# haosulab/ActiveZero

Measured on AMD Instinct MI355X. Metric: stereo pairs/sec (540x960, D=192) fwd+bwd, higher is better.
Workload: dtype f32; 1 GPU; configs[1]: PSMNet 540x960 (padded to 544 rows) D=192 fwd+bwd+Adam, supervised disparity loss, batch 4 per GPU; global_batch=4, height=540, width=960, maxdisp=192, parallelism=dp1

## Files before the change

### activezero_amd/csrc/az_conv3d_c1.hip

```cpp
#include "az_common.h"

#define C1_TH 8
#define C1_TW 32
#define C1_VS 36
#define C1_GP 36
typedef float c1_f2 __attribute__((ext_vector_type(2)));
#define C1_FMA2(a, b, c) __builtin_elementwise_fma(a, b, c)


#define C1F_TH 8
#define C1F_TW 16
template <int CTRL>
__device__ __forceinline__ float c1_dpp_add(float v) {
    return v + __builtin_bit_cast(float, __builtin_amdgcn_update_dpp(0, __builtin_bit_cast(int, v), CTRL, 0xf, 0xf, true));
}
__global__ void __launch_bounds__(256)
c1_fwd_kernel(float *__restrict__ out, const float *__restrict__ in, const float *__restrict__ w,
              const float *__restrict__ addend, const float *__restrict__ in_scale,
              const float *__restrict__ in_shift, int D, int H, int W, int tiles_x, int dseg) {
    constexpr int SX = C1F_TW + 2, SY = C1F_TH + 2;
    __shared__ __attribute__((aligned(16))) float slab[SY * SX * C1_VS];
    const int tx0 = (blockIdx.x % tiles_x) * C1F_TW, ty0 = (blockIdx.x / tiles_x) * C1F_TH;
    const int d0 = blockIdx.y * dseg, d1 = min(d0 + dseg, D), b = blockIdx.z;
    const int cp = threadIdx.x & 15, grp = threadIdx.x >> 4;
    const int ly = grp >> 1, lx0 = (grp & 1) * 8;
    const int oh = ty0 + ly;
    c1_f2 wp[27];
#pragma unroll
    for (int t = 0; t < 27; ++t) wp[t] = c1_f2{w[(cp * 2 + 0) * 27 + t], w[(cp * 2 + 1) * 27 + t]};
    c1_f2 a_prev[8], a_cur[8], a_next[8];
#pragma unroll
    for (int j = 0; j < 8; ++j) { a_prev[j] = c1_f2{0.f, 0.f}; a_cur[j] = c1_f2{0.f, 0.f}; a_next[j] = c1_f2{0.f, 0.f}; }
    constexpr int NQ = SY * SX * 8, NLD = (NQ + 255) / 256;
    float4 pre[NLD];
    const bool affine = in_scale != nullptr;
    float4 isc = make_float4(1.f, 1.f, 1.f, 1.f), ish = make_float4(0.f, 0.f, 0.f, 0.f);
    if (affine) {
        isc = reinterpret_cast<const float4 *>(in_scale)[threadIdx.x & 7];
        ish = reinterpret_cast<const float4 *>(in_shift)[threadIdx.x & 7];
    }
    unsigned okbits = 0;
    auto issue = [&](int id) {
        okbits = 0;
#pragma unroll
        for (int it = 0; it < NLD; ++it) {
            const int q = threadIdx.x + 256 * it, v = q >> 3, part = q & 7;
            const int sy = v / SX, sx = v - sy * SX;
            const int ih = ty0 - 1 + sy, iw = tx0 - 1 + sx;
            pre[it] = make_float4(0.f, 0.f, 0.f, 0.f);
            if (q < NQ && id >= 0 && id < D && ih >= 0 && ih < H && iw >= 0 && iw < W) {
                pre[it] = *reinterpret_cast<const float4 *>(
                    in + ((((size_t)b * D + id) * H + ih) * W + iw) * 32 + part * 4);
                okbits |= 1u << it;
            }
        }
    };
    issue(d0 - 1);
    for (int id = d0 - 1; id <= d1; ++id) {
        if (id >= 0 && id < D) {
            __syncthreads();
#pragma unroll
            for (int it = 0; it < NLD; ++it) {
                const int q = threadIdx.x + 256 * it;
                float4 v = pre[it];
                if (affine && ((okbits >> it) & 1u)) {
                    v.x = fmaxf(fmaf(v.x, isc.x, ish.x), 0.f); v.y = fmaxf(fmaf(v.y, isc.y, ish.y), 0.f);
                    v.z = fmaxf(fmaf(v.z, isc.z, ish.z), 0.f); v.w = fmaxf(fmaf(v.w, isc.w, ish.w), 0.f);
                }
                if (q < NQ) *reinterpret_cast<float4 *>(&slab[(q >> 3) * C1_VS + (q & 7) * 4]) = v;
            }
            __syncthreads();
        }
        if (id < d1) issue(id + 1);
        if (id >= 0 && id < D) {
#pragma unroll
            for (int kh = 0; kh < 3; ++kh) {
                c1_f2 r[10];
                const float *row = &slab[((ly + kh) * SX + lx0) * C1_VS + cp * 2];
#pragma unroll
                for (int i = 0; i < 10; ++i) {
                    const float2 x = *reinterpret_cast<const float2 *>(row + i * C1_VS);
                    r[i] = c1_f2{x.x, x.y};
                }
#pragma unroll
                for (int kw = 0; kw < 3; ++kw)
#pragma unroll
                    for (int j = 0; j < 8; ++j) {
                        a_next[j] = C1_FMA2(r[j + kw], wp[kh * 3 + kw], a_next[j]);
                        a_cur[j] = C1_FMA2(r[j + kw], wp[9 + kh * 3 + kw], a_cur[j]);
                        a_prev[j] = C1_FMA2(r[j + kw], wp[18 + kh * 3 + kw], a_prev[j]);
                    }
            }
        }
        const int od = id - 1;
        if (od >= d0 && od < d1) {
            float mine = 0.f;
#pragma unroll
            for (int j = 0; j < 8; ++j) {
                float v = a_prev[j][0] + a_prev[j][1];
                v = c1_dpp_add<0xB1>(v);
                v = c1_dpp_add<0x4E>(v);
                v = c1_dpp_add<0x141>(v);
                v = c1_dpp_add<0x140>(v);
                mine = (cp == j) ? v : mine;
            }
            const int ow = tx0 + lx0 + cp;
            if (cp < 8 && oh < H && ow < W) {
                const size_t o = (((size_t)b * D + od) * H + oh) * W + ow;
                out[o] = addend ? mine + addend[o] : mine;
            }
        }
#pragma unroll
        for (int j = 0; j < 8; ++j) { a_prev[j] = a_cur[j]; a_cur[j] = a_next[j]; a_next[j] = c1_f2{0.f, 0.f}; }
    }
}

__device__ __forceinline__ void c1_load_gtile(float *gt, const float *__restrict__ gout, int b,
                                              int od, int ty0, int tx0, int D, int H, int W) {
    constexpr int SX = C1_TW + 2, SY = C1_TH + 2;
    for (int q = threadIdx.x; q < 3 * SY * SX; q += 256) {
        const int sx = q % SX;
        const int r = q / SX;
        const int sy = r % SY, sd = r / SY;
        const int gd = od - 1 + sd, gh = ty0 - 1 + sy, gw = tx0 - 1 + sx;
        gt[r * C1_GP + sx] = (gd >= 0 && gd < D && gh >= 0 && gh < H && gw >= 0 && gw < W)
                                 ? gout[(((size_t)b * D + gd) * H + gh) * W + gw] : 0.f;
    }
}
__device__ __forceinline__ void c1_row6(float (&r)[6], const float *gt, int pd, int sy, int lx0) {
    const float *row = static_cast<const float *>(__builtin_assume_aligned(gt + (pd * (C1_TH + 2) + sy) * C1_GP + lx0, 16));
    const float4 a = *reinterpret_cast<const float4 *>(row);
    const float2 c = *reinterpret_cast<const float2 *>(row + 4);
    r[0] = a.x; r[1] = a.y; r[2] = a.z; r[3] = a.w; r[4] = c.x; r[5] = c.y;
}

__global__ void __launch_bounds__(256)
c1_dgrad_kernel(float *__restrict__ gin, const float *__restrict__ gout,
                const float *__restrict__ w, int D, int H, int W, int tiles_x) {
    constexpr int SY = C1_TH + 2;
    __shared__ __attribute__((aligned(16))) float gt[3 * SY * C1_GP];
    const int tx0 = (blockIdx.x % tiles_x) * C1_TW, ty0 = (blockIdx.x / tiles_x) * C1_TH;
    const int od = blockIdx.y, b = blockIdx.z;
    c1_load_gtile(gt, gout, b, od, ty0, tx0, D, H, W);
    const int cp = threadIdx.x & 15, grp = threadIdx.x >> 4;
    c1_f2 wp[27];
#pragma unroll
    for (int t = 0; t < 27; ++t) wp[t] = c1_f2{w[(cp * 2 + 0) * 27 + t], w[(cp * 2 + 1) * 27 + t]};
    __syncthreads();
#pragma unroll 1
    for (int p = 0; p < C1_TH * C1_TW / 128; ++p) {
        const int gi = p * 16 + grp, ly = gi >> 2, lx0 = (gi & 3) * 8;
        const int oh = ty0 + ly;
        c1_f2 acc[8];
#pragma unroll
        for (int j = 0; j < 8; ++j) acc[j] = c1_f2{0.f, 0.f};
#pragma unroll
        for (int kd = 0; kd < 3; ++kd)
#pragma unroll
            for (int kh = 0; kh < 3; ++kh) {
                float r[12];
                {
                    const float *row = static_cast<const float *>(__builtin_assume_aligned(
                        gt + ((2 - kd) * SY + ly + 2 - kh) * C1_GP + lx0, 16));
                    const float4 a = *reinterpret_cast<const float4 *>(row);
                    const float4 c = *reinterpret_cast<const float4 *>(row + 4);
                    const float2 e = *reinterpret_cast<const float2 *>(row + 8);
                    r[0] = a.x; r[1] = a.y; r[2] = a.z; r[3] = a.w; r[4] = c.x; r[5] = c.y; r[6] = c.z; r[7] = c.w;
                    r[8] = e.x; r[9] = e.y;
                }
#pragma unroll
                for (int kw = 0; kw < 3; ++kw) {
                    const int t = (kd * 3 + kh) * 3 + kw;
#pragma unroll
                    for (int j = 0; j < 8; ++j) {
                        const c1_f2 g2 = {r[j + 2 - kw], r[j + 2 - kw]};
                        acc[j] = C1_FMA2(g2, wp[t], acc[j]);
                    }
                }
            }
#pragma unroll
        for (int j = 0; j < 8; ++j) asm volatile("" : "+v"(acc[j]));
        if (oh < H) {
            float *dst = gin + ((((size_t)b * D + od) * H + oh) * W + tx0 + lx0) * 32 + cp * 2;
#pragma unroll
            for (int j = 0; j < 8; ++j)
                if (tx0 + lx0 + j < W) *reinterpret_cast<float2 *>(dst + j * 32) = make_float2(acc[j][0], acc[j][1]);
        }
    }
}

__global__ void __launch_bounds__(256)
c1_wgrad_kernel(float *__restrict__ gw, const float *__restrict__ in,
                const float *__restrict__ gout, const float *__restrict__ in_scale,
                const float *__restrict__ in_shift, int D, int H, int W, int tiles_x, int tiles_y,
                long long ntiles) {
    constexpr int SY = C1_TH + 2;
    __shared__ __attribute__((aligned(16))) float gt[3 * SY * C1_GP];
    __shared__ float red[864];
    for (int q = threadIdx.x; q < 864; q += 256) red[q] = 0.f;
    const int quad = threadIdx.x & 7, grp = threadIdx.x >> 3;
    const bool affine = in_scale != nullptr;
    float4 isc = make_float4(1.f, 1.f, 1.f, 1.f), ish = make_float4(0.f, 0.f, 0.f, 0.f);
    if (affine) {
        isc = reinterpret_cast<const float4 *>(in_scale)[quad];
        ish = reinterpret_cast<const float4 *>(in_shift)[quad];
    }
    c1_f2 a01[27], a23[27];
#pragma unroll
    for (int t = 0; t < 27; ++t) { a01[t] = c1_f2{0.f, 0.f}; a23[t] = c1_f2{0.f, 0.f}; }
    for (long long item = blockIdx.x; item < ntiles; item += gridDim.x) {
        long long r = item;
        const int tx0 = (int)(r % tiles_x) * C1_TW; r /= tiles_x;
        const int ty0 = (int)(r % tiles_y) * C1_TH; r /= tiles_y;
        const int od = (int)(r % D);
        const int b = (int)(r / D);
        __syncthreads();
        c1_load_gtile(gt, gout, b, od, ty0, tx0, D, H, W);
        __syncthreads();
#pragma unroll 1
        for (int p = 0; p < C1_TH * C1_TW / 128; ++p) {
            const int gi = p * 32 + grp, ly = gi >> 3, lx0 = (gi & 7) * 4;
            const int ih = ty0 + ly;
            c1_f2 x01[4], x23[4];
            const float *src = in + ((((size_t)b * D + od) * H + ih) * W + tx0 + lx0) * 32 + quad * 4;
#pragma unroll
            for (int j = 0; j < 4; ++j) {
                float4 x = make_float4(0.f, 0.f, 0.f, 0.f);
                if (ih < H && tx0 + lx0 + j < W) {
                    x = *reinterpret_cast<const float4 *>(src + j * 32);
                    if (affine) {
                        x.x = fmaxf(fmaf(x.x, isc.x, ish.x), 0.f); x.y = fmaxf(fmaf(x.y, isc.y, ish.y), 0.f);
                        x.z = fmaxf(fmaf(x.z, isc.z, ish.z), 0.f); x.w = fmaxf(fmaf(x.w, isc.w, ish.w), 0.f);
                    }
                }
                x01[j] = c1_f2{x.x, x.y}; x23[j] = c1_f2{x.z, x.w};
            }
#pragma unroll
            for (int kd = 0; kd < 3; ++kd)
#pragma unroll
                for (int kh = 0; kh < 3; ++kh) {
                    float r[6];
                    c1_row6(r, gt, 2 - kd, ly + 2 - kh, lx0);
#pragma unroll
                    for (int kw = 0; kw < 3; ++kw) {
                        const int t = (kd * 3 + kh) * 3 + kw;
#pragma unroll
                        for (int j = 0; j < 4; ++j) {
                            const c1_f2 g2 = {r[j + 2 - kw], r[j + 2 - kw]};
                            a01[t] = C1_FMA2(g2, x01[j], a01[t]);
                            a23[t] = C1_FMA2(g2, x23[j], a23[t]);
                        }
                    }
                }
        }
    }
#pragma unroll
    for (int c = 0; c < 4; ++c)
#pragma unroll
        for (int t = 0; t < 27; ++t) {
            float v = (c < 2 ? a01[t] : a23[t])[c & 1];
            v += __shfl_xor(v, 8); v += __shfl_xor(v, 16); v += __shfl_xor(v, 32);
            if ((threadIdx.x & 63) < 8) atomicAdd(&red[(quad * 4 + c) * 27 + t], v);
        }
    __syncthreads();
    for (int q = threadIdx.x; q < 864; q += 256) atomicAdd(&gw[q], red[q]);
}

static int c1_check(int B, int D, int H, int W) {
    if (!(B > 0 && D > 0 && H > 0 && W > 0)) return AZ_EINVAL;
    if (B > 65535 || D > 65535) return AZ_EUNSUPPORTED;
    return AZ_OK;
}

extern "C" int az_conv3d_c1_fwd(float *logits, const float *in, const float *w,
                                const float *addend, const float *in_scale, const float *in_shift, int B, int D,
                                int H, int W, void *stream) {
    AZ_REQUIRE_PTR(logits); AZ_REQUIRE_PTR(in); AZ_REQUIRE_PTR(w);
    if ((in_scale == nullptr) != (in_shift == nullptr)) return AZ_EINVAL;
    if (int e = c1_check(B, D, H, W)) return e;
    const int tiles_x = (W + C1F_TW - 1) / C1F_TW, tiles_y = (H + C1F_TH - 1) / C1F_TH;
    int best = 1;
    long long best_cost = -1;
    for (int nseg = 1; nseg <= D; ++nseg) {
        const int dseg = (D + nseg - 1) / nseg;
        const long long blocks = (long long)tiles_x * tiles_y * B * ((D + dseg - 1) / dseg);
        const long long cost = ((blocks + 767) / 768) * (dseg + 2);
        if (best_cost < 0 || cost < best_cost) { best_cost = cost; best = dseg; }
    }
    hipLaunchKernelGGL(c1_fwd_kernel, dim3(tiles_x * tiles_y, (D + best - 1) / best, B), dim3(256), 0,
                       az_stream(stream), logits, in, w, addend, in_scale, in_shift, D, H, W, tiles_x, best);
    return az_launch_status();
}

extern "C" int az_conv3d_c1_dgrad(float *grad_in, const float *grad_logits, const float *w,
                                  int B, int D, int H, int W, void *stream) {
    AZ_REQUIRE_PTR(grad_in); AZ_REQUIRE_PTR(grad_logits); AZ_REQUIRE_PTR(w);
    if (int e = c1_check(B, D, H, W)) return e;
    const int tiles_x = (W + C1_TW - 1) / C1_TW, tiles_y = (H + C1_TH - 1) / C1_TH;
    hipLaunchKernelGGL(c1_dgrad_kernel, dim3(tiles_x * tiles_y, D, B), dim3(256), 0,
                       az_stream(stream), grad_in, grad_logits, w, D, H, W, tiles_x);
    return az_launch_status();
}

extern "C" int az_conv3d_c1_wgrad(float *grad_w, const float *in, const float *grad_logits,
                                  const float *in_scale, const float *in_shift, int B, int D, int H, int W,
                                  void *stream) {
    AZ_REQUIRE_PTR(grad_w); AZ_REQUIRE_PTR(in); AZ_REQUIRE_PTR(grad_logits);
    if ((in_scale == nullptr) != (in_shift == nullptr)) return AZ_EINVAL;
    if (int e = c1_check(B, D, H, W)) return e;
    if (hipMemsetAsync(grad_w, 0, 864 * sizeof(float), az_stream(stream)) != hipSuccess)
        return AZ_ELAUNCH;
    const int tiles_x = (W + C1_TW - 1) / C1_TW, tiles_y = (H + C1_TH - 1) / C1_TH;
    const long long ntiles = (long long)B * D * tiles_y * tiles_x;
    const unsigned grid = (unsigned)(ntiles < 2048 ? ntiles : 2048);
    hipLaunchKernelGGL(c1_wgrad_kernel, dim3(grid), dim3(256), 0, az_stream(stream), grad_w, in,
                       grad_logits, in_scale, in_shift, D, H, W, tiles_x, tiles_y, ntiles);
    return az_launch_status();
}
```

### activezero_amd/csrc/az_softargmin.hip

```cpp
#include "az_common.h"

#define SA_TY 4
#define SA_TX 64
#define SA_LY 3
#define SA_LX 18

__device__ __forceinline__ void sa_load_tile(float *tile, const float *__restrict__ logits,
                                             int b, int d, int h, int w, int ybase, int xbase) {
    const int n = d * SA_LY * SA_LX;
    for (int e = threadIdx.x; e < n; e += blockDim.x) {
        const int lx = e % SA_LX;
        const int r = e / SA_LX;
        const int ly = r % SA_LY, k = r / SA_LY;
        const int gy = min(max(ybase + ly, 0), h - 1);
        const int gx = min(max(xbase + lx, 0), w - 1);
        tile[e] = logits[(((size_t)b * d + k) * h + gy) * w + gx];
    }
}

__device__ __forceinline__ float sa_exp_fast(float x) { return __builtin_amdgcn_exp2f(x * 1.4426950408889634f); }

struct SaPix {
    int ly0, lx0;
    float wy1, wx1;
};

__device__ __forceinline__ void sa_axis(int dst, int base, int &l0, float &lam1) {
    const int q = dst >> 2, r = dst & 3;
    l0 = ((r < 2) ? q - 1 : q) - base;
    lam1 = (r < 2) ? (r == 0 ? 0.625f : 0.875f) : (r == 2 ? 0.125f : 0.375f);
}

__device__ __forceinline__ float sa_plane(const float *tile, int k, const SaPix &p) {
    const float *t = tile + k * (SA_LY * SA_LX);
    const float *c = t + p.ly0 * SA_LX + p.lx0;
    const float a00 = c[0], a01 = c[1], a10 = c[SA_LX], a11 = c[SA_LX + 1];
    const float wx0 = 1.f - p.wx1, wy0 = 1.f - p.wy1;
    return wy0 * (wx0 * a00 + p.wx1 * a01) + p.wy1 * (wx0 * a10 + p.wx1 * a11);
}

template <int DP>
__device__ __forceinline__ void sa_stats_planes(const float *tile, const SaPix &p, float &M, float &s, float &t) {
    float v[DP];
#pragma unroll
    for (int k = 0; k < DP; ++k) v[k] = sa_plane(tile, k, p);
    M = fmaxf(v[0], v[DP - 1]);
#pragma unroll
    for (int k = 0; k + 1 < DP; ++k)
        M = fmaxf(M, fmaxf(0.875f * v[k] + 0.125f * v[k + 1], 0.125f * v[k] + 0.875f * v[k + 1]));
#pragma unroll
    for (int k = 0; k < DP; ++k) v[k] = (v[k] - M) * 1.4426950408889634f;
    float sa[4] = {0.f, 0.f, 0.f, 0.f}, ta[4] = {0.f, 0.f, 0.f, 0.f};
    {
        const float e = __builtin_amdgcn_exp2f(v[0]);
        sa[0] += e + e;
        ta[0] += e;
    }
#pragma unroll
    for (int k = 0; k + 1 < DP; ++k) {
#pragma unroll
        for (int m = 0; m < 4; ++m) {
            const float w1 = 0.125f + 0.25f * m;
            const float e = __builtin_amdgcn_exp2f((1.f - w1) * v[k] + w1 * v[k + 1]);
            sa[m] += e;
            ta[m] = fmaf((float)(4 * k + 2 + m), e, ta[m]);
        }
    }
    {
        const float e = __builtin_amdgcn_exp2f(v[DP - 1]);
        sa[1] += e + e;
        ta[1] += (float)(4 * DP - 2) * e + (float)(4 * DP - 1) * e;
    }
    s = (sa[0] + sa[1]) + (sa[2] + sa[3]);
    t = (ta[0] + ta[1]) + (ta[2] + ta[3]);
}

__device__ __forceinline__ void sa_stats(const float *tile, int d, const SaPix &p, float &M,
                                         float &s, float &t) {
    if (d == 48) { sa_stats_planes<48>(tile, p, M, s, t); return; }
    if (d == 16) { sa_stats_planes<16>(tile, p, M, s, t); return; }
    {
        float a0 = sa_plane(tile, 0, p);
        M = a0;
        for (int k = 0; k + 1 < d; ++k) {
            const float a1 = sa_plane(tile, k + 1, p);
            M = fmaxf(M, fmaxf(0.875f * a0 + 0.125f * a1, 0.125f * a0 + 0.875f * a1));
            a0 = a1;
        }
        M = fmaxf(M, a0);
    }
    const float L2E = 1.4426950408889634f;
    s = 0.f;
    t = 0.f;
    float v0 = (sa_plane(tile, 0, p) - M) * L2E;
    {
        const float e = __builtin_amdgcn_exp2f(v0);
        s += e + e;
        t += e;
    }
    for (int k = 0; k + 1 < d; ++k) {
        const float v1 = (sa_plane(tile, k + 1, p) - M) * L2E;
#pragma unroll
        for (int m = 0; m < 4; ++m) {
            const float w1 = 0.125f + 0.25f * m;
            const float e = __builtin_amdgcn_exp2f((1.f - w1) * v0 + w1 * v1);
            s += e;
            t = fmaf((float)(4 * k + 2 + m), e, t);
        }
        v0 = v1;
    }
    {
        const float e = __builtin_amdgcn_exp2f(v0);
        s += e + e;
        t += (float)(4 * d - 2) * e + (float)(4 * d - 1) * e;
    }
}

__global__ void __launch_bounds__(256)
softargmin_fwd_kernel(float *__restrict__ out, float2 *__restrict__ stats,
                      const float *__restrict__ logits, int d, int h, int w, int tiles_x) {
    extern __shared__ float tile[];
    const int H = 4 * h, W = 4 * w;
    const int tx = blockIdx.x % tiles_x, ty = blockIdx.x / tiles_x;
    const int b = blockIdx.y;
    const int ybase = ty * (SA_TY / 4) - 1, xbase = tx * (SA_TX / 4) - 1;
    sa_load_tile(tile, logits, b, d, h, w, ybase, xbase);
    __syncthreads();
    const int Y = ty * SA_TY + (threadIdx.x >> 6), X = tx * SA_TX + (threadIdx.x & 63);
    if (X >= W || Y >= H) return;
    SaPix p;
    sa_axis(Y, ybase, p.ly0, p.wy1);
    sa_axis(X, xbase, p.lx0, p.wx1);
    float M, s, t;
    sa_stats(tile, d, p, M, s, t);
    out[((size_t)b * H + Y) * W + X] = t / s;
    if (stats) stats[((size_t)b * H + Y) * W + X] = make_float2(M, s);
}

__global__ void __launch_bounds__(256)
softargmin_bwd_kernel(float *__restrict__ glogits, const float *__restrict__ gout,
                      const float *__restrict__ logits, const float2 *__restrict__ stats,
                      const float *__restrict__ fwd_out, int d, int h, int w, int tiles_x) {
    extern __shared__ float smem[];
    float *tile = smem;
    float *gtile = smem + d * SA_LY * SA_LX;
    float *gmine = gtile + (threadIdx.x >> 6) * (d * 2 * SA_LX);
    const int H = 4 * h, W = 4 * w;
    const int tx = blockIdx.x % tiles_x, ty = blockIdx.x / tiles_x;
    const int b = blockIdx.y;
    const int ybase = ty * (SA_TY / 4) - 1, xbase = tx * (SA_TX / 4) - 1;
    const int ncell = d * SA_LY * SA_LX;
    sa_load_tile(tile, logits, b, d, h, w, ybase, xbase);
    __syncthreads();
    const int Y = ty * SA_TY + (threadIdx.x >> 6), X = tx * SA_TX + (threadIdx.x & 63);
    const bool live = (X < W) && (Y < H);
    SaPix p;
    sa_axis(Y, ybase, p.ly0, p.wy1);
    sa_axis(X, xbase, p.lx0, p.wx1);
    float M, s, pred;
    if (stats) {
        const size_t pix = live ? ((size_t)b * H + Y) * W + X : 0;
        const float2 ms = stats[pix];
        M = ms.x; s = ms.y; pred = fwd_out[pix];
    } else {
        float t;
        sa_stats(tile, d, p, M, s, t);
        pred = t / s;
    }
    const float g = live ? gout[((size_t)b * H + Y) * W + X] / s : 0.f;

    const int r = threadIdx.x & 3, wl = threadIdx.x & 63;
    const int cq = (X >> 2) - xbase;
    const float wx0 = 1.f - p.wx1;
    const float f_m1 = (r < 2) ? wx0 : 0.f;
    const float f_0 = (r < 2) ? p.wx1 : wx0;
    const float f_p1 = (r < 2) ? 0.f : p.wx1;

    float v0 = sa_plane(tile, 0, p);
    float acc0;
    {
        const float e = sa_exp_fast(v0 - M);
        acc0 = g * e * ((0.f - pred) + (1.f - pred));
    }
    for (int k = 0; k < d; ++k) {
        float acc1 = 0.f;
        if (k + 1 < d) {
            const float v1 = sa_plane(tile, k + 1, p);
#pragma unroll
            for (int m = 0; m < 4; ++m) {
                const float w1 = 0.125f + 0.25f * m;
                const float u = (1.f - w1) * v0 + w1 * v1;
                const float gu = g * sa_exp_fast(u - M) * ((float)(4 * k + 2 + m) - pred);
                acc0 += (1.f - w1) * gu;
                acc1 += w1 * gu;
            }
            v0 = v1;
        } else {
            const float e = sa_exp_fast(v0 - M);
            acc0 += g * e * (((float)(4 * d - 2) - pred) + ((float)(4 * d - 1) - pred));
        }
        float s_m1 = f_m1 * acc0, s_0 = f_0 * acc0, s_p1 = f_p1 * acc0;
        s_m1 += __shfl_xor(s_m1, 1); s_m1 += __shfl_xor(s_m1, 2);
        s_0 += __shfl_xor(s_0, 1);   s_0 += __shfl_xor(s_0, 2);
        s_p1 += __shfl_xor(s_p1, 1); s_p1 += __shfl_xor(s_p1, 2);
        const float from_left = __shfl_up(s_p1, 4), from_right = __shfl_down(s_m1, 4);
        const float cell = s_0 + (wl >= 4 ? from_left : 0.f) + (wl < 60 ? from_right : 0.f);
        const bool edge_l = (wl == 1), edge_r = (wl == 61);
        if (r == 0 || edge_l || edge_r) {
            const float val = (r == 0) ? cell : (edge_l ? s_m1 : s_p1);
            const int col = (r == 0) ? cq : (edge_l ? cq - 1 : cq + 1);
            float *gt = gmine + k * (2 * SA_LX) + col;
            gt[0] = (1.f - p.wy1) * val;
            gt[SA_LX] = p.wy1 * val;
        }
        acc0 = acc1;
    }
    __syncthreads();
    int ly0_of[SA_TY];
#pragma unroll
    for (int wv = 0; wv < SA_TY; ++wv) {
        SaPix q;
        sa_axis(ty * SA_TY + wv, ybase, q.ly0, q.wy1);
        ly0_of[wv] = q.ly0;
    }
    for (int e = threadIdx.x; e < ncell; e += blockDim.x) {
        const int lx = e % SA_LX;
        const int rr = e / SA_LX;
        const int ly = rr % SA_LY, k = rr / SA_LY;
        float v = 0.f;
#pragma unroll
        for (int wv = 0; wv < SA_TY; ++wv) {
            const int slot = ly - ly0_of[wv];
            if (slot == 0 || slot == 1) v += gtile[(wv * d + k) * (2 * SA_LX) + slot * SA_LX + lx];
        }
        if (v == 0.f) continue;
        const int gy = min(max(ybase + ly, 0), h - 1);
        const int gx = min(max(xbase + lx, 0), w - 1);
        atomicAdd(&glogits[(((size_t)b * d + k) * h + gy) * w + gx], v);
    }
}

static int sa_check(int B, int d, int h, int w) {
    if (!(B > 0 && d > 0 && h > 0 && w > 0)) return AZ_EINVAL;
    if (B > 65535) return AZ_EUNSUPPORTED;
    if (((size_t)d * SA_LY * SA_LX + (size_t)SA_TY * d * 2 * SA_LX) * sizeof(float) > 64 * 1024) return AZ_EUNSUPPORTED;
    return AZ_OK;
}

extern "C" int az_softargmin_fwd(float *disp_out, float *stats_out, const float *logits, int B, int d,
                                 int h, int w, void *stream) {
    AZ_REQUIRE_PTR(disp_out); AZ_REQUIRE_PTR(logits);
    if (int e = sa_check(B, d, h, w)) return e;
    const int tiles_x = (4 * w + SA_TX - 1) / SA_TX, tiles_y = (4 * h) / SA_TY;
    hipLaunchKernelGGL(softargmin_fwd_kernel, dim3(tiles_x * tiles_y, B), dim3(256),
                       (size_t)d * SA_LY * SA_LX * sizeof(float), az_stream(stream), disp_out,
                       reinterpret_cast<float2 *>(stats_out), logits, d, h, w, tiles_x);
    return az_launch_status();
}

extern "C" int az_softargmin_bwd(float *grad_logits, const float *grad_disp,
                                 const float *logits, const float *stats, const float *disp_fwd,
                                 int B, int d, int h, int w, void *stream) {
    AZ_REQUIRE_PTR(grad_logits); AZ_REQUIRE_PTR(grad_disp); AZ_REQUIRE_PTR(logits);
    if ((stats == nullptr) != (disp_fwd == nullptr)) return AZ_EINVAL;
    if (int e = sa_check(B, d, h, w)) return e;
    if (hipMemsetAsync(grad_logits, 0, (size_t)B * d * h * w * sizeof(float),
                       az_stream(stream)) != hipSuccess)
        return AZ_ELAUNCH;
    const int tiles_x = (4 * w + SA_TX - 1) / SA_TX, tiles_y = (4 * h) / SA_TY;
    hipLaunchKernelGGL(softargmin_bwd_kernel, dim3(tiles_x * tiles_y, B), dim3(256),
                       ((size_t)d * SA_LY * SA_LX + (size_t)SA_TY * d * 2 * SA_LX) * sizeof(float), az_stream(stream),
                       grad_logits, grad_disp, logits, reinterpret_cast<const float2 *>(stats), disp_fwd,
                       d, h, w, tiles_x);
    return az_launch_status();
}
```

Before: 47.87 pairs/s.

## Double-buffer conv3d c1 kernels, segment dgrad depth, retile softargmin backward

The c1 forward kernel now double-buffers its LDS slab, so staging the next depth plane overlaps compute and each iteration needs one barrier instead of two. The dgrad kernel walks a depth segment with a 4-plane ring buffer and register prefetch, where before it launched one block per output depth and reloaded three planes each time. The wgrad kernel prefetches its next input tile into registers. The depth-segment heuristic is moved into a shared helper that assumes 256 CUs. The softargmin backward processes four output rows per thread over a taller tile and may request more than 64KB of LDS, which lowers occupancy and adds code complexity.

```diff
diff --git a/activezero_amd/csrc/az_conv3d_c1.hip b/activezero_amd/csrc/az_conv3d_c1.hip
--- a/activezero_amd/csrc/az_conv3d_c1.hip
+++ b/activezero_amd/csrc/az_conv3d_c1.hip
@@ -18,8 +18,8 @@
 c1_fwd_kernel(float *__restrict__ out, const float *__restrict__ in, const float *__restrict__ w,
               const float *__restrict__ addend, const float *__restrict__ in_scale,
               const float *__restrict__ in_shift, int D, int H, int W, int tiles_x, int dseg) {
-    constexpr int SX = C1F_TW + 2, SY = C1F_TH + 2;
-    __shared__ __attribute__((aligned(16))) float slab[SY * SX * C1_VS];
+    constexpr int SX = C1F_TW + 2, SY = C1F_TH + 2, SLAB = SY * SX * C1_VS;
+    __shared__ __attribute__((aligned(16))) float slab[2 * SLAB];
     const int tx0 = (blockIdx.x % tiles_x) * C1F_TW, ty0 = (blockIdx.x / tiles_x) * C1F_TH;
     const int d0 = blockIdx.y * dseg, d1 = min(d0 + dseg, D), b = blockIdx.z;
     const int cp = threadIdx.x & 15, grp = threadIdx.x >> 4;
@@ -55,28 +55,34 @@
             }
         }
     };
+    auto stage = [&](int buf) {
+#pragma unroll
+        for (int it = 0; it < NLD; ++it) {
+            const int q = threadIdx.x + 256 * it;
+            float4 v = pre[it];
+            if (affine && ((okbits >> it) & 1u)) {
+                v.x = fmaxf(fmaf(v.x, isc.x, ish.x), 0.f); v.y = fmaxf(fmaf(v.y, isc.y, ish.y), 0.f);
+                v.z = fmaxf(fmaf(v.z, isc.z, ish.z), 0.f); v.w = fmaxf(fmaf(v.w, isc.w, ish.w), 0.f);
+            }
+            if (q < NQ) *reinterpret_cast<float4 *>(&slab[buf * SLAB + (q >> 3) * C1_VS + (q & 7) * 4]) = v;
+        }
+    };
     issue(d0 - 1);
-    for (int id = d0 - 1; id <= d1; ++id) {
+    if (d0 - 1 >= 0) stage(0);
+    issue(d0);
+    int buf = 0;
+    for (int id = d0 - 1; id <= d1; ++id, buf ^= 1) {
+        __syncthreads();
+        if (id < d1) {
+            if (id + 1 < D) stage(buf ^ 1);
+            if (id + 1 < d1) issue(id + 2);
+        }
         if (id >= 0 && id < D) {
-            __syncthreads();
-#pragma unroll
-            for (int it = 0; it < NLD; ++it) {
-                const int q = threadIdx.x + 256 * it;
-                float4 v = pre[it];
-                if (affine && ((okbits >> it) & 1u)) {
-                    v.x = fmaxf(fmaf(v.x, isc.x, ish.x), 0.f); v.y = fmaxf(fmaf(v.y, isc.y, ish.y), 0.f);
-                    v.z = fmaxf(fmaf(v.z, isc.z, ish.z), 0.f); v.w = fmaxf(fmaf(v.w, isc.w, ish.w), 0.f);
-                }
-                if (q < NQ) *reinterpret_cast<float4 *>(&slab[(q >> 3) * C1_VS + (q & 7) * 4]) = v;
-            }
-            __syncthreads();
-        }
-        if (id < d1) issue(id + 1);
-        if (id >= 0 && id < D) {
+            const float *pl = slab + buf * SLAB;
 #pragma unroll
             for (int kh = 0; kh < 3; ++kh) {
                 c1_f2 r[10];
-                const float *row = &slab[((ly + kh) * SX + lx0) * C1_VS + cp * 2];
+                const float *row = &pl[((ly + kh) * SX + lx0) * C1_VS + cp * 2];
 #pragma unroll
                 for (int i = 0; i < 10; ++i) {
                     const float2 x = *reinterpret_cast<const float2 *>(row + i * C1_VS);
@@ -136,56 +142,85 @@
 
 __global__ void __launch_bounds__(256)
 c1_dgrad_kernel(float *__restrict__ gin, const float *__restrict__ gout,
-                const float *__restrict__ w, int D, int H, int W, int tiles_x) {
-    constexpr int SY = C1_TH + 2;
-    __shared__ __attribute__((aligned(16))) float gt[3 * SY * C1_GP];
+                const float *__restrict__ w, int D, int H, int W, int tiles_x, int dseg) {
+    constexpr int SX = C1_TW + 2, SY = C1_TH + 2, PL = SY * C1_GP;
+    constexpr int NG = (SY * SX + 255) / 256;
+    __shared__ __attribute__((aligned(16))) float gt[4 * PL];
     const int tx0 = (blockIdx.x % tiles_x) * C1_TW, ty0 = (blockIdx.x / tiles_x) * C1_TH;
-    const int od = blockIdx.y, b = blockIdx.z;
-    c1_load_gtile(gt, gout, b, od, ty0, tx0, D, H, W);
+    const int d0 = blockIdx.y * dseg, d1 = min(d0 + dseg, D), b = blockIdx.z;
+    float pre[NG];
+    auto issue = [&](int gd) {
+#pragma unroll
+        for (int it = 0; it < NG; ++it) {
+            const int q = threadIdx.x + 256 * it;
+            const int sy = q / SX, sx = q - sy * SX;
+            const int gh = ty0 - 1 + sy, gw = tx0 - 1 + sx;
+            pre[it] = (q < SY * SX && gd >= 0 && gd < D && gh >= 0 && gh < H && gw >= 0 && gw < W)
+                          ? gout[(((size_t)b * D + gd) * H + gh) * W + gw] : 0.f;
+        }
+    };
+    auto stage = [&](int gd) {
+        float *pl = gt + ((gd + 1) & 3) * PL;
+#pragma unroll
+        for (int it = 0; it < NG; ++it) {
+            const int q = threadIdx.x + 256 * it;
+            const int sy = q / SX, sx = q - sy * SX;
+            if (q < SY * SX) pl[sy * C1_GP + sx] = pre[it];
+        }
+    };
+    issue(d0 - 1); stage(d0 - 1);
+    issue(d0); stage(d0);
+    issue(d0 + 1); stage(d0 + 1);
     const int cp = threadIdx.x & 15, grp = threadIdx.x >> 4;
     c1_f2 wp[27];
 #pragma unroll
     for (int t = 0; t < 27; ++t) wp[t] = c1_f2{w[(cp * 2 + 0) * 27 + t], w[(cp * 2 + 1) * 27 + t]};
-    __syncthreads();
 #pragma unroll 1
-    for (int p = 0; p < C1_TH * C1_TW / 128; ++p) {
-        const int gi = p * 16 + grp, ly = gi >> 2, lx0 = (gi & 3) * 8;
-        const int oh = ty0 + ly;
-        c1_f2 acc[8];
-#pragma unroll
-        for (int j = 0; j < 8; ++j) acc[j] = c1_f2{0.f, 0.f};
-#pragma unroll
-        for (int kd = 0; kd < 3; ++kd)
-#pragma unroll
-            for (int kh = 0; kh < 3; ++kh) {
-                float r[12];
-                {
-                    const float *row = static_cast<const float *>(__builtin_assume_aligned(
-                        gt + ((2 - kd) * SY + ly + 2 - kh) * C1_GP + lx0, 16));
-                    const float4 a = *reinterpret_cast<const float4 *>(row);
-                    const float4 c = *reinterpret_cast<const float4 *>(row + 4);
-                    const float2 e = *reinterpret_cast<const float2 *>(row + 8);
-                    r[0] = a.x; r[1] = a.y; r[2] = a.z; r[3] = a.w; r[4] = c.x; r[5] = c.y; r[6] = c.z; r[7] = c.w;
-                    r[8] = e.x; r[9] = e.y;
-                }
-#pragma unroll
-                for (int kw = 0; kw < 3; ++kw) {
-                    const int t = (kd * 3 + kh) * 3 + kw;
-#pragma unroll
-                    for (int j = 0; j < 8; ++j) {
-                        const c1_f2 g2 = {r[j + 2 - kw], r[j + 2 - kw]};
-                        acc[j] = C1_FMA2(g2, wp[t], acc[j]);
+    for (int od = d0; od < d1; ++od) {
+        __syncthreads();
+        const bool more = od + 1 < d1;
+        if (more) issue(od + 2);
+#pragma unroll 1
+        for (int p = 0; p < C1_TH * C1_TW / 128; ++p) {
+            const int gi = p * 16 + grp, ly = gi >> 2, lx0 = (gi & 3) * 8;
+            const int oh = ty0 + ly;
+            c1_f2 acc[8];
+#pragma unroll
+            for (int j = 0; j < 8; ++j) acc[j] = c1_f2{0.f, 0.f};
+#pragma unroll
+            for (int kd = 0; kd < 3; ++kd)
+#pragma unroll
+                for (int kh = 0; kh < 3; ++kh) {
+                    float r[12];
+                    {
+                        const float *row = static_cast<const float *>(__builtin_assume_aligned(
+                            gt + ((od + 2 - kd) & 3) * PL + (ly + 2 - kh) * C1_GP + lx0, 16));
+                        const float4 a = *reinterpret_cast<const float4 *>(row);
+                        const float4 c = *reinterpret_cast<const float4 *>(row + 4);
+                        const float2 e = *reinterpret_cast<const float2 *>(row + 8);
+                        r[0] = a.x; r[1] = a.y; r[2] = a.z; r[3] = a.w; r[4] = c.x; r[5] = c.y; r[6] = c.z; r[7] = c.w;
+                        r[8] = e.x; r[9] = e.y;
+                    }
+#pragma unroll
+                    for (int kw = 0; kw < 3; ++kw) {
+                        const int t = (kd * 3 + kh) * 3 + kw;
+#pragma unroll
+                        for (int j = 0; j < 8; ++j) {
+                            const c1_f2 g2 = {r[j + 2 - kw], r[j + 2 - kw]};
+                            acc[j] = C1_FMA2(g2, wp[t], acc[j]);
+                        }
                     }
                 }
-            }
-#pragma unroll
-        for (int j = 0; j < 8; ++j) asm volatile("" : "+v"(acc[j]));
-        if (oh < H) {
-            float *dst = gin + ((((size_t)b * D + od) * H + oh) * W + tx0 + lx0) * 32 + cp * 2;
-#pragma unroll
-            for (int j = 0; j < 8; ++j)
-                if (tx0 + lx0 + j < W) *reinterpret_cast<float2 *>(dst + j * 32) = make_float2(acc[j][0], acc[j][1]);
-        }
+#pragma unroll
+            for (int j = 0; j < 8; ++j) asm volatile("" : "+v"(acc[j]));
+            if (oh < H) {
+                float *dst = gin + ((((size_t)b * D + od) * H + oh) * W + tx0 + lx0) * 32 + cp * 2;
+#pragma unroll
+                for (int j = 0; j < 8; ++j)
+                    if (tx0 + lx0 + j < W) *reinterpret_cast<float2 *>(dst + j * 32) = make_float2(acc[j][0], acc[j][1]);
+            }
+        }
+        if (more) stage(od + 2);
     }
 }
 
@@ -208,32 +243,60 @@
     c1_f2 a01[27], a23[27];
 #pragma unroll
     for (int t = 0; t < 27; ++t) { a01[t] = c1_f2{0.f, 0.f}; a23[t] = c1_f2{0.f, 0.f}; }
+    auto locate = [&](long long item, int &tx0, int &ty0, int &od, int &b) {
+        long long r = item;
+        tx0 = (int)(r % tiles_x) * C1_TW; r /= tiles_x;
+        ty0 = (int)(r % tiles_y) * C1_TH; r /= tiles_y;
+        od = (int)(r % D);
+        b = (int)(r / D);
+    };
+    float4 nxt[4];
+    unsigned nok = 0;
+    auto fetch = [&](int tx0, int ty0, int od, int b, int p, bool any) {
+        const int gi = p * 32 + grp, ly = gi >> 3, lx0 = (gi & 7) * 4;
+        const int ih = ty0 + ly;
+        const float *src = in + ((((size_t)b * D + od) * H + ih) * W + tx0 + lx0) * 32 + quad * 4;
+        nok = 0;
+#pragma unroll
+        for (int j = 0; j < 4; ++j) {
+            nxt[j] = make_float4(0.f, 0.f, 0.f, 0.f);
+            if (any && ih < H && tx0 + lx0 + j < W) {
+                nxt[j] = *reinterpret_cast<const float4 *>(src + j * 32);
+                nok |= 1u << j;
+            }
+        }
+    };
+    {
+        int tx0, ty0, od, b;
+        locate(blockIdx.x, tx0, ty0, od, b);
+        fetch(tx0, ty0, od, b, 0, (long long)blockIdx.x < ntiles);
+    }
     for (long long item = blockIdx.x; item < ntiles; item += gridDim.x) {
-        long long r = item;
-        const int tx0 = (int)(r % tiles_x) * C1_TW; r /= tiles_x;
-        const int ty0 = (int)(r % tiles_y) * C1_TH; r /= tiles_y;
-        const int od = (int)(r % D);
-        const int b = (int)(r / D);
+        int tx0, ty0, od, b;
+        locate(item, tx0, ty0, od, b);
         __syncthreads();
         c1_load_gtile(gt, gout, b, od, ty0, tx0, D, H, W);
         __syncthreads();
 #pragma unroll 1
         for (int p = 0; p < C1_TH * C1_TW / 128; ++p) {
             const int gi = p * 32 + grp, ly = gi >> 3, lx0 = (gi & 7) * 4;
-            const int ih = ty0 + ly;
             c1_f2 x01[4], x23[4];
-            const float *src = in + ((((size_t)b * D + od) * H + ih) * W + tx0 + lx0) * 32 + quad * 4;
 #pragma unroll
             for (int j = 0; j < 4; ++j) {
-                float4 x = make_float4(0.f, 0.f, 0.f, 0.f);
-                if (ih < H && tx0 + lx0 + j < W) {
-                    x = *reinterpret_cast<const float4 *>(src + j * 32);
-                    if (affine) {
-                        x.x = fmaxf(fmaf(x.x, isc.x, ish.x), 0.f); x.y = fmaxf(fmaf(x.y, isc.y, ish.y), 0.f);
-                        x.z = fmaxf(fmaf(x.z, isc.z, ish.z), 0.f); x.w = fmaxf(fmaf(x.w, isc.w, ish.w), 0.f);
-                    }
+                float4 x = nxt[j];
+                if (affine && ((nok >> j) & 1u)) {
+                    x.x = fmaxf(fmaf(x.x, isc.x, ish.x), 0.f); x.y = fmaxf(fmaf(x.y, isc.y, ish.y), 0.f);
+                    x.z = fmaxf(fmaf(x.z, isc.z, ish.z), 0.f); x.w = fmaxf(fmaf(x.w, isc.w, ish.w), 0.f);
                 }
                 x01[j] = c1_f2{x.x, x.y}; x23[j] = c1_f2{x.z, x.w};
+            }
+            if (p + 1 < C1_TH * C1_TW / 128) {
+                fetch(tx0, ty0, od, b, p + 1, true);
+            } else {
+                int ntx0, nty0, nod, nb;
+                const long long nitem = item + gridDim.x;
+                locate(nitem < ntiles ? nitem : item, ntx0, nty0, nod, nb);
+                fetch(ntx0, nty0, nod, nb, 0, nitem < ntiles);
             }
 #pragma unroll
             for (int kd = 0; kd < 3; ++kd)
@@ -266,6 +329,19 @@
     for (int q = threadIdx.x; q < 864; q += 256) atomicAdd(&gw[q], red[q]);
 }
 
+#define C1_CUS 256
+static int c1_depth_segment(long long tiles, int D, int halo) {
+    int best = 1;
+    long long best_cost = -1;
+    for (int nseg = 1; nseg <= D; ++nseg) {
+        const int dseg = (D + nseg - 1) / nseg;
+        const long long blocks = tiles * ((D + dseg - 1) / dseg);
+        const long long cost = ((blocks + C1_CUS - 1) / C1_CUS) * (dseg + halo);
+        if (best_cost < 0 || cost < best_cost) { best_cost = cost; best = dseg; }
+    }
+    return best;
+}
+
 static int c1_check(int B, int D, int H, int W) {
     if (!(B > 0 && D > 0 && H > 0 && W > 0)) return AZ_EINVAL;
     if (B > 65535 || D > 65535) return AZ_EUNSUPPORTED;
@@ -279,14 +355,7 @@
     if ((in_scale == nullptr) != (in_shift == nullptr)) return AZ_EINVAL;
     if (int e = c1_check(B, D, H, W)) return e;
     const int tiles_x = (W + C1F_TW - 1) / C1F_TW, tiles_y = (H + C1F_TH - 1) / C1F_TH;
-    int best = 1;
-    long long best_cost = -1;
-    for (int nseg = 1; nseg <= D; ++nseg) {
-        const int dseg = (D + nseg - 1) / nseg;
-        const long long blocks = (long long)tiles_x * tiles_y * B * ((D + dseg - 1) / dseg);
-        const long long cost = ((blocks + 767) / 768) * (dseg + 2);
-        if (best_cost < 0 || cost < best_cost) { best_cost = cost; best = dseg; }
-    }
+    const int best = c1_depth_segment((long long)tiles_x * tiles_y * B, D, 2);
     hipLaunchKernelGGL(c1_fwd_kernel, dim3(tiles_x * tiles_y, (D + best - 1) / best, B), dim3(256), 0,
                        az_stream(stream), logits, in, w, addend, in_scale, in_shift, D, H, W, tiles_x, best);
     return az_launch_status();
@@ -297,8 +366,9 @@
     AZ_REQUIRE_PTR(grad_in); AZ_REQUIRE_PTR(grad_logits); AZ_REQUIRE_PTR(w);
     if (int e = c1_check(B, D, H, W)) return e;
     const int tiles_x = (W + C1_TW - 1) / C1_TW, tiles_y = (H + C1_TH - 1) / C1_TH;
-    hipLaunchKernelGGL(c1_dgrad_kernel, dim3(tiles_x * tiles_y, D, B), dim3(256), 0,
-                       az_stream(stream), grad_in, grad_logits, w, D, H, W, tiles_x);
+    const int dseg = c1_depth_segment((long long)tiles_x * tiles_y * B, D, 1);
+    hipLaunchKernelGGL(c1_dgrad_kernel, dim3(tiles_x * tiles_y, (D + dseg - 1) / dseg, B), dim3(256), 0,
+                       az_stream(stream), grad_in, grad_logits, w, D, H, W, tiles_x, dseg);
     return az_launch_status();
 }
 
diff --git a/activezero_amd/csrc/az_softargmin.hip b/activezero_amd/csrc/az_softargmin.hip
--- a/activezero_amd/csrc/az_softargmin.hip
+++ b/activezero_amd/csrc/az_softargmin.hip
@@ -4,14 +4,18 @@
 #define SA_TX 64
 #define SA_LY 3
 #define SA_LX 18
-
+#define SAB_TY 16
+#define SAB_LY 6
+#define SA_SCALAR(x) asm volatile("" : "+v"(x))
+
+template <int LY>
 __device__ __forceinline__ void sa_load_tile(float *tile, const float *__restrict__ logits,
                                              int b, int d, int h, int w, int ybase, int xbase) {
-    const int n = d * SA_LY * SA_LX;
+    const int n = d * LY * SA_LX;
     for (int e = threadIdx.x; e < n; e += blockDim.x) {
         const int lx = e % SA_LX;
         const int r = e / SA_LX;
-        const int ly = r % SA_LY, k = r / SA_LY;
+        const int ly = r % LY, k = r / LY;
         const int gy = min(max(ybase + ly, 0), h - 1);
         const int gx = min(max(xbase + lx, 0), w - 1);
         tile[e] = logits[(((size_t)b * d + k) * h + gy) * w + gx];
@@ -31,19 +35,20 @@
     lam1 = (r < 2) ? (r == 0 ? 0.625f : 0.875f) : (r == 2 ? 0.125f : 0.375f);
 }
 
+template <int LY>
 __device__ __forceinline__ float sa_plane(const float *tile, int k, const SaPix &p) {
-    const float *t = tile + k * (SA_LY * SA_LX);
+    const float *t = tile + k * (LY * SA_LX);
     const float *c = t + p.ly0 * SA_LX + p.lx0;
     const float a00 = c[0], a01 = c[1], a10 = c[SA_LX], a11 = c[SA_LX + 1];
     const float wx0 = 1.f - p.wx1, wy0 = 1.f - p.wy1;
     return wy0 * (wx0 * a00 + p.wx1 * a01) + p.wy1 * (wx0 * a10 + p.wx1 * a11);
 }
 
-template <int DP>
+template <int DP, int LY>
 __device__ __forceinline__ void sa_stats_planes(const float *tile, const SaPix &p, float &M, float &s, float &t) {
     float v[DP];
 #pragma unroll
-    for (int k = 0; k < DP; ++k) v[k] = sa_plane(tile, k, p);
+    for (int k = 0; k < DP; ++k) v[k] = sa_plane<LY>(tile, k, p);
     M = fmaxf(v[0], v[DP - 1]);
 #pragma unroll
     for (int k = 0; k + 1 < DP; ++k)
@@ -75,15 +80,16 @@
     t = (ta[0] + ta[1]) + (ta[2] + ta[3]);
 }
 
+template <int LY>
 __device__ __forceinline__ void sa_stats(const float *tile, int d, const SaPix &p, float &M,
                                          float &s, float &t) {
-    if (d == 48) { sa_stats_planes<48>(tile, p, M, s, t); return; }
-    if (d == 16) { sa_stats_planes<16>(tile, p, M, s, t); return; }
-    {
-        float a0 = sa_plane(tile, 0, p);
+    if (d == 48) { sa_stats_planes<48, LY>(tile, p, M, s, t); return; }
+    if (d == 16) { sa_stats_planes<16, LY>(tile, p, M, s, t); return; }
+    {
+        float a0 = sa_plane<LY>(tile, 0, p);
         M = a0;
         for (int k = 0; k + 1 < d; ++k) {
-            const float a1 = sa_plane(tile, k + 1, p);
+            const float a1 = sa_plane<LY>(tile, k + 1, p);
             M = fmaxf(M, fmaxf(0.875f * a0 + 0.125f * a1, 0.125f * a0 + 0.875f * a1));
             a0 = a1;
         }
@@ -92,14 +98,14 @@
     const float L2E = 1.4426950408889634f;
     s = 0.f;
     t = 0.f;
-    float v0 = (sa_plane(tile, 0, p) - M) * L2E;
+    float v0 = (sa_plane<LY>(tile, 0, p) - M) * L2E;
     {
         const float e = __builtin_amdgcn_exp2f(v0);
         s += e + e;
         t += e;
     }
     for (int k = 0; k + 1 < d; ++k) {
-        const float v1 = (sa_plane(tile, k + 1, p) - M) * L2E;
+        const float v1 = (sa_plane<LY>(tile, k + 1, p) - M) * L2E;
 #pragma unroll
         for (int m = 0; m < 4; ++m) {
             const float w1 = 0.125f + 0.25f * m;
@@ -124,7 +130,7 @@
     const int tx = blockIdx.x % tiles_x, ty = blockIdx.x / tiles_x;
     const int b = blockIdx.y;
     const int ybase = ty * (SA_TY / 4) - 1, xbase = tx * (SA_TX / 4) - 1;
-    sa_load_tile(tile, logits, b, d, h, w, ybase, xbase);
+    sa_load_tile<SA_LY>(tile, logits, b, d, h, w, ybase, xbase);
     __syncthreads();
     const int Y = ty * SA_TY + (threadIdx.x >> 6), X = tx * SA_TX + (threadIdx.x & 63);
     if (X >= W || Y >= H) return;
@@ -132,7 +138,7 @@
     sa_axis(Y, ybase, p.ly0, p.wy1);
     sa_axis(X, xbase, p.lx0, p.wx1);
     float M, s, t;
-    sa_stats(tile, d, p, M, s, t);
+    sa_stats<SA_LY>(tile, d, p, M, s, t);
     out[((size_t)b * H + Y) * W + X] = t / s;
     if (stats) stats[((size_t)b * H + Y) * W + X] = make_float2(M, s);
 }
@@ -143,95 +149,128 @@
                       const float *__restrict__ fwd_out, int d, int h, int w, int tiles_x) {
     extern __shared__ float smem[];
     float *tile = smem;
-    float *gtile = smem + d * SA_LY * SA_LX;
-    float *gmine = gtile + (threadIdx.x >> 6) * (d * 2 * SA_LX);
+    const int ncell = d * SAB_LY * SA_LX;
+    float *gtile = smem + ncell;
+    const int wv = threadIdx.x >> 6;
+    float *gmine = gtile + wv * (d * 3 * SA_LX);
     const int H = 4 * h, W = 4 * w;
     const int tx = blockIdx.x % tiles_x, ty = blockIdx.x / tiles_x;
     const int b = blockIdx.y;
-    const int ybase = ty * (SA_TY / 4) - 1, xbase = tx * (SA_TX / 4) - 1;
-    const int ncell = d * SA_LY * SA_LX;
-    sa_load_tile(tile, logits, b, d, h, w, ybase, xbase);
+    const int ybase = ty * (SAB_TY / 4) - 1, xbase = tx * (SA_TX / 4) - 1;
+    sa_load_tile<SAB_LY>(tile, logits, b, d, h, w, ybase, xbase);
     __syncthreads();
-    const int Y = ty * SA_TY + (threadIdx.x >> 6), X = tx * SA_TX + (threadIdx.x & 63);
-    const bool live = (X < W) && (Y < H);
-    SaPix p;
-    sa_axis(Y, ybase, p.ly0, p.wy1);
-    sa_axis(X, xbase, p.lx0, p.wx1);
-    float M, s, pred;
-    if (stats) {
-        const size_t pix = live ? ((size_t)b * H + Y) * W + X : 0;
-        const float2 ms = stats[pix];
-        M = ms.x; s = ms.y; pred = fwd_out[pix];
-    } else {
-        float t;
-        sa_stats(tile, d, p, M, s, t);
-        pred = t / s;
-    }
-    const float g = live ? gout[((size_t)b * H + Y) * W + X] / s : 0.f;
-
-    const int r = threadIdx.x & 3, wl = threadIdx.x & 63;
-    const int cq = (X >> 2) - xbase;
-    const float wx0 = 1.f - p.wx1;
-    const float f_m1 = (r < 2) ? wx0 : 0.f;
-    const float f_0 = (r < 2) ? p.wx1 : wx0;
-    const float f_p1 = (r < 2) ? 0.f : p.wx1;
-
-    float v0 = sa_plane(tile, 0, p);
-    float acc0;
-    {
-        const float e = sa_exp_fast(v0 - M);
-        acc0 = g * e * ((0.f - pred) + (1.f - pred));
-    }
-    for (int k = 0; k < d; ++k) {
-        float acc1 = 0.f;
-        if (k + 1 < d) {
-            const float v1 = sa_plane(tile, k + 1, p);
-#pragma unroll
-            for (int m = 0; m < 4; ++m) {
-                const float w1 = 0.125f + 0.25f * m;
-                const float u = (1.f - w1) * v0 + w1 * v1;
-                const float gu = g * sa_exp_fast(u - M) * ((float)(4 * k + 2 + m) - pred);
-                acc0 += (1.f - w1) * gu;
-                acc1 += w1 * gu;
+    const int qy = ty * (SAB_TY / 4) + wv, X = tx * SA_TX + (threadIdx.x & 63);
+    if (qy < h) {
+        const bool live = X < W;
+        SaPix p[4];
+#pragma unroll
+        for (int j = 0; j < 4; ++j) {
+            sa_axis(4 * qy + j, ybase, p[j].ly0, p[j].wy1);
+            sa_axis(X, xbase, p[j].lx0, p[j].wx1);
+        }
+        float M[4], g[4], pred[4];
+#pragma unroll
+        for (int j = 0; j < 4; ++j) {
+            const size_t pix = live ? ((size_t)b * H + 4 * qy + j) * W + X : 0;
+            float s;
+            if (stats) {
+                const float2 ms = stats[pix];
+                M[j] = ms.x; s = ms.y; pred[j] = fwd_out[pix];
+            } else {
+                float t;
+                sa_stats<SAB_LY>(tile, d, p[j], M[j], s, t);
+                pred[j] = t / s;
             }
-            v0 = v1;
-        } else {
-            const float e = sa_exp_fast(v0 - M);
-            acc0 += g * e * (((float)(4 * d - 2) - pred) + ((float)(4 * d - 1) - pred));
-        }
-        float s_m1 = f_m1 * acc0, s_0 = f_0 * acc0, s_p1 = f_p1 * acc0;
-        s_m1 += __shfl_xor(s_m1, 1); s_m1 += __shfl_xor(s_m1, 2);
-        s_0 += __shfl_xor(s_0, 1);   s_0 += __shfl_xor(s_0, 2);
-        s_p1 += __shfl_xor(s_p1, 1); s_p1 += __shfl_xor(s_p1, 2);
-        const float from_left = __shfl_up(s_p1, 4), from_right = __shfl_down(s_m1, 4);
-        const float cell = s_0 + (wl >= 4 ? from_left : 0.f) + (wl < 60 ? from_right : 0.f);
+            g[j] = live ? gout[pix] / s : 0.f;
+        }
+
+        const int r = threadIdx.x & 3, wl = threadIdx.x & 63;
+        const int cq = (X >> 2) - xbase;
+        const float wx1 = p[0].wx1, wx0 = 1.f - wx1;
+        const float f_m1 = (r < 2) ? wx0 : 0.f;
+        const float f_0 = (r < 2) ? wx1 : wx0;
+        const float f_p1 = (r < 2) ? 0.f : wx1;
         const bool edge_l = (wl == 1), edge_r = (wl == 61);
-        if (r == 0 || edge_l || edge_r) {
-            const float val = (r == 0) ? cell : (edge_l ? s_m1 : s_p1);
-            const int col = (r == 0) ? cq : (edge_l ? cq - 1 : cq + 1);
-            float *gt = gmine + k * (2 * SA_LX) + col;
-            gt[0] = (1.f - p.wy1) * val;
-            gt[SA_LX] = p.wy1 * val;
-        }
-        acc0 = acc1;
+        const bool writer = (r == 0) || edge_l || edge_r;
+        const int col = (r == 0) ? cq : (edge_l ? cq - 1 : cq + 1);
+        auto put = [&](float val, float *dst) {
+            float s_m1 = f_m1 * val, s_0 = f_0 * val, s_p1 = f_p1 * val;
+            s_m1 += __shfl_xor(s_m1, 1); s_m1 += __shfl_xor(s_m1, 2);
+            s_0 += __shfl_xor(s_0, 1);   s_0 += __shfl_xor(s_0, 2);
+            s_p1 += __shfl_xor(s_p1, 1); s_p1 += __shfl_xor(s_p1, 2);
+            const float from_left = __shfl_up(s_p1, 4), from_right = __shfl_down(s_m1, 4);
+            const float cell = s_0 + (wl >= 4 ? from_left : 0.f) + (wl < 60 ? from_right : 0.f);
+            if (writer) dst[col] = (r == 0) ? cell : (edge_l ? s_m1 : s_p1);
+        };
+        const float *cbase = tile + wv * SA_LX + p[0].lx0;
+        auto planes = [&](int k, float (&v)[4]) {
+            const float *c = cbase + k * (SAB_LY * SA_LX);
+            float hx[3];
+#pragma unroll
+            for (int rr = 0; rr < 3; ++rr) hx[rr] = wx0 * c[rr * SA_LX] + wx1 * c[rr * SA_LX + 1];
+#pragma unroll
+            for (int j = 0; j < 4; ++j) {
+                v[j] = (1.f - p[j].wy1) * hx[j >> 1] + p[j].wy1 * hx[(j >> 1) + 1];
+                SA_SCALAR(v[j]);
+            }
+        };
+
+        float v0[4], acc0[4];
+        planes(0, v0);
+#pragma unroll
+        for (int j = 0; j < 4; ++j) {
+            const float e = sa_exp_fast(v0[j] - M[j]);
+            float d0 = 0.f - pred[j];
+            SA_SCALAR(d0);
+            acc0[j] = g[j] * e * (d0 + (1.f - pred[j]));
+        }
+        for (int k = 0; k < d; ++k) {
+            float acc1[4] = {0.f, 0.f, 0.f, 0.f};
+            if (k + 1 < d) {
+                float v1[4];
+                planes(k + 1, v1);
+#pragma unroll
+                for (int j = 0; j < 4; ++j) {
+#pragma unroll
+                    for (int m = 0; m < 4; ++m) {
+                        const float w1 = 0.125f + 0.25f * m;
+                        const float u = (1.f - w1) * v0[j] + w1 * v1[j];
+                        float gu = g[j] * sa_exp_fast(u - M[j]) * ((float)(4 * k + 2 + m) - pred[j]);
+                        SA_SCALAR(gu);
+                        acc0[j] += (1.f - w1) * gu;
+                        acc1[j] += w1 * gu;
+                    }
+                    v0[j] = v1[j];
+                    SA_SCALAR(acc0[j]); SA_SCALAR(acc1[j]);
+                }
+            } else {
+#pragma unroll
+                for (int j = 0; j < 4; ++j) {
+                    const float e = sa_exp_fast(v0[j] - M[j]);
+                    float dl = (float)(4 * d - 2) - pred[j];
+                    SA_SCALAR(dl);
+                    acc0[j] += g[j] * e * (dl + ((float)(4 * d - 1) - pred[j]));
+                }
+            }
+            float *gk = gmine + k * (3 * SA_LX);
+            put((1.f - p[0].wy1) * acc0[0] + (1.f - p[1].wy1) * acc0[1], gk);
+            put((p[0].wy1 * acc0[0] + p[1].wy1 * acc0[1]) + ((1.f - p[2].wy1) * acc0[2] + (1.f - p[3].wy1) * acc0[3]),
+                gk + SA_LX);
+            put(p[2].wy1 * acc0[2] + p[3].wy1 * acc0[3], gk + 2 * SA_LX);
+#pragma unroll
+            for (int j = 0; j < 4; ++j) acc0[j] = acc1[j];
+        }
     }
     __syncthreads();
-    int ly0_of[SA_TY];
-#pragma unroll
-    for (int wv = 0; wv < SA_TY; ++wv) {
-        SaPix q;
-        sa_axis(ty * SA_TY + wv, ybase, q.ly0, q.wy1);
-        ly0_of[wv] = q.ly0;
-    }
     for (int e = threadIdx.x; e < ncell; e += blockDim.x) {
         const int lx = e % SA_LX;
         const int rr = e / SA_LX;
-        const int ly = rr % SA_LY, k = rr / SA_LY;
+        const int ly = rr % SAB_LY, k = rr / SAB_LY;
         float v = 0.f;
 #pragma unroll
-        for (int wv = 0; wv < SA_TY; ++wv) {
-            const int slot = ly - ly0_of[wv];
-            if (slot == 0 || slot == 1) v += gtile[(wv * d + k) * (2 * SA_LX) + slot * SA_LX + lx];
+        for (int wq = 0; wq < SAB_TY / 4; ++wq) {
+            const int slot = ly - wq;
+            if (slot >= 0 && slot < 3 && ty * (SAB_TY / 4) + wq < h) v += gtile[(wq * d + k) * (3 * SA_LX) + slot * SA_LX + lx];
         }
         if (v == 0.f) continue;
         const int gy = min(max(ybase + ly, 0), h - 1);
@@ -240,10 +279,12 @@
     }
 }
 
+static size_t sa_bwd_lds(int d) { return ((size_t)d * SAB_LY * SA_LX + (size_t)(SAB_TY / 4) * d * 3 * SA_LX) * sizeof(float); }
+
 static int sa_check(int B, int d, int h, int w) {
     if (!(B > 0 && d > 0 && h > 0 && w > 0)) return AZ_EINVAL;
     if (B > 65535) return AZ_EUNSUPPORTED;
-    if (((size_t)d * SA_LY * SA_LX + (size_t)SA_TY * d * 2 * SA_LX) * sizeof(float) > 64 * 1024) return AZ_EUNSUPPORTED;
+    if (sa_bwd_lds(d) > 160 * 1024) return AZ_EUNSUPPORTED;
     return AZ_OK;
 }
 
@@ -264,12 +305,16 @@
     AZ_REQUIRE_PTR(grad_logits); AZ_REQUIRE_PTR(grad_disp); AZ_REQUIRE_PTR(logits);
     if ((stats == nullptr) != (disp_fwd == nullptr)) return AZ_EINVAL;
     if (int e = sa_check(B, d, h, w)) return e;
+    const size_t lds = sa_bwd_lds(d);
+    if (lds > 64 * 1024 &&
+        hipFuncSetAttribute(reinterpret_cast<const void *>(softargmin_bwd_kernel),
+                            hipFuncAttributeMaxDynamicSharedMemorySize, (int)lds) != hipSuccess)
+        return AZ_EUNSUPPORTED;
     if (hipMemsetAsync(grad_logits, 0, (size_t)B * d * h * w * sizeof(float),
                        az_stream(stream)) != hipSuccess)
         return AZ_ELAUNCH;
-    const int tiles_x = (4 * w + SA_TX - 1) / SA_TX, tiles_y = (4 * h) / SA_TY;
-    hipLaunchKernelGGL(softargmin_bwd_kernel, dim3(tiles_x * tiles_y, B), dim3(256),
-                       ((size_t)d * SA_LY * SA_LX + (size_t)SA_TY * d * 2 * SA_LX) * sizeof(float), az_stream(stream),
+    const int tiles_x = (4 * w + SA_TX - 1) / SA_TX, tiles_y = (4 * h + SAB_TY - 1) / SAB_TY;
+    hipLaunchKernelGGL(softargmin_bwd_kernel, dim3(tiles_x * tiles_y, B), dim3(256), lds, az_stream(stream),
                        grad_logits, grad_disp, logits, reinterpret_cast<const float2 *>(stats), disp_fwd,
                        d, h, w, tiles_x);
     return az_launch_status();
```

New measurement: 48.12 pairs/s (median of 6 runs). Within noise of the previous version (+0.5%).
